# martius-lab/iCEM

Measured on AMD Instinct MI355X. Metric: traj-steps/sec (N x h), iCEM inner planning loop, higher is better.
Workload: dtype f32 storage; model step 2xfp16 planes (3 products), f32 accumulate

## Files before the change

### icem_amd/csrc/fused_dev.h

```cpp
#pragma once
#include "icem_fused.h"

#include <climits>
#include <cmath>
#include <cstdlib>
#include <algorithm>
#include <type_traits>
#include <utility>

#include "exchange_dev.h"
#include "philox.h"
#include "refit.h"

#ifndef ICEM_FAST_SHAPES
#define ICEM_FAST_SHAPES(X) X(30, 6, 17) X(30, 6, 18) X(12, 6, 17) X(13, 4, 17) X(30, 17, 24)
#endif
#define ICEM_FAST_HORIZONS(X) X(30) X(12) X(13) X(10)

namespace icem {

namespace {

constexpr int HMAX = 32;
constexpr int SWG = 256;
// ... 1459 lines not shown
        n_cand += (unsigned)__popcll(m);
    }
    __builtin_amdgcn_fence(__ATOMIC_SEQ_CST, "workgroup");
    if (n_cand <= 64) {
        unsigned long long key = lane < (int)n_cand ? lds_reread_u64(&cand[lane]) : KEY_SENTINEL;
        key = wave_sort_n(key, lane, n_cand);
        if (lane < a.K) sel[lane] = key;
    } else {
        for (int r = 0; r < a.K; ++r) {
            unsigned long long head = k[0];
#pragma unroll
            for (int j = 1; j < 5; ++j) head = k[j] < head ? k[j] : head;
            const unsigned long long best = wave_min_u64(head);
            if (best != KEY_SENTINEL) {
#pragma unroll
                for (int j = 0; j < 5; ++j)
                    if (k[j] == best) k[j] = KEY_SENTINEL;
            }
            if (lane == 0) sel[r] = best;
        }
    }
}

template <int NW>
__device__ __forceinline__ bool merge_select_split_by_rank(const MergeSingleArgs& a) { return a.n_keep <= (16 - a.K) * NW; }
template <int NW>
__device__ __forceinline__ float merge_keep_cost_split(const MergeSingleArgs& a, int lane, int w) {
    const int j = w + NW * (lane - a.K);
    return a.elites_cost_cur ? a.elites_cost_cur[(lane >= a.K && lane < 16 && j < a.n_keep) ? j : 0] : 0.f;
}
template <int NW>
__device__ __forceinline__ void merge_select_split_keep(const MergeSingleArgs& a, int lane, int w, unsigned long long* wsel,
                                                        unsigned long long* sel, float keep_cost) {
    if (lane >= a.K && lane < 16) {
        const int j = w + NW * (lane - a.K);
        wsel[w * 16 + lane] = (j < a.n_keep && a.elites_cost_cur) ? make_key(keep_cost, keep_index0(a) + j) : KEY_SENTINEL;
    }
    if (w == 0 && lane < 16) sel[lane] = KEY_SENTINEL;
}
template <int NW>
__device__ __forceinline__ void merge_select_split_rank(const MergeSingleArgs& a, int lane, int w, const unsigned long long* wsel,
                                                        unsigned long long* sel) {
    typedef unsigned long long u64x2 __attribute__((ext_vector_type(2)));
    const int i = lane & 15, q = lane >> 4;
    const unsigned long long mine = wsel[w * 16 + i];
    const u64x2* pairs = reinterpret_cast<const u64x2*>(wsel) + q;
    unsigned place = 0;
#pragma unroll
    for (int c = 0; c < 2 * NW; ++c) {
        const u64x2 b = pairs[4 * c];
        place += (b[0] < mine ? 1u : 0u) + (b[1] < mine ? 1u : 0u);
    }
    place += (unsigned)__shfl_xor((int)place, 16, 64);
    place += (unsigned)__shfl_xor((int)place, 32, 64);
    if (q == 0 && mine != KEY_SENTINEL && place < (unsigned)a.K) sel[place] = mine;
}

template <int KREG, bool REC>
__device__ __forceinline__ void merge_rows(const MergeSingleArgs& a, const unsigned long long* sel, const int* slot,
                                           const float* (&rows)[KREG]) {
    const int hd = a.h * a.d;
    const int lane = (int)(threadIdx.x & 63);
    const int v = REC ? slot[lane < a.K ? lane : 0] : key_idx(sel[lane < a.K ? lane : 0]);
    const float* mine;
    if (REC) mine = v < a.n_rec ? a.records + (size_t)v * (hd + 2) + 2 : a.elites_cur + (size_t)(v - a.n_rec) * hd;
    else mine = v < a.n_pool ? a.actions + (size_t)v * hd : a.elites_cur + (size_t)(v - a.n_global) * hd;
    typedef const float __attribute__((address_space(1))) * GRow;
    const unsigned long long bits = (unsigned long long)(size_t)mine;
#pragma unroll
    for (int r = 0; r < KREG; ++r) {
        const int rr = r < a.K ? r : 0;
        const unsigned lo = (unsigned)__builtin_amdgcn_readlane((int)(unsigned)bits, rr);
        const unsigned hi = (unsigned)__builtin_amdgcn_readlane((int)(unsigned)(bits >> 32), rr);
        rows[r] = (const float*)reinterpret_cast<GRow>((size_t)(((unsigned long long)hi << 32) | lo));
    }
}

template <int H, int D, int ROUNDS, bool RAW>
__device__ __forceinline__ void sample_into_tile(const FastSampleArgs& sa, int n_rows, int r_mine, int jd, float* trow,
                                                 const float* mrow) {
    constexpr int HD = H * D;
    if (r_mine < sa.n) {
        if (RAW) {
            sample_row<H, ROUNDS>(sa.W, (unsigned)(sa.first_index + r_mine), (unsigned)jd, sa.off_lo, sa.off_hi,
                                  sa.seed_lo, sa.seed_hi, [&](int t, float y) { trow[t * D] = y; }, sa.white != 0);
        } else {
            const float lo = sa.low[jd], hi = sa.high[jd];
            sample_row<H, ROUNDS>(sa.W, (unsigned)(sa.first_index + r_mine), (unsigned)jd, sa.off_lo, sa.off_hi,
                                  sa.seed_lo, sa.seed_hi, [&](int t, float y) {
                                      const float v = __builtin_fmaf(y, mrow[HD + t * D], mrow[t * D]);
                                      trow[t * D] = __builtin_amdgcn_fmed3f(v, lo, hi);
                                  }, sa.white != 0);
        }
    } else if (r_mine < n_rows && !RAW) {
        const int e = r_mine - sa.n;
        const float lo = sa.low[jd], hi = sa.high[jd];
        float last = 0.f;
        sample_row<H, ROUNDS>(sa.W, (unsigned)e, (unsigned)jd, sa.off2_lo, sa.off2_hi, sa.seed_lo, sa.seed_hi,
                              [&](int t, float y) {
                                  if (t == H - 1) {
                                      const float v = __builtin_fmaf(y, mrow[HD + t * D], mrow[t * D]);
                                      last = __builtin_amdgcn_fmed3f(v, lo, hi);
                                  }
                              }, sa.white != 0);
        const float* src = sa.elites_src + (size_t)e * HD + jd;
        for (int t = 0; t < H - 1; ++t) trow[t * D] = src[(t + 1) * D];
        trow[(H - 1) * D] = last;
    } else {
        for (int t = 0; t < H; ++t) trow[t * D] = 0.f;
    }
}

template <int H, int D, int ROUNDS, bool RAW, typename Publish>
__device__ __forceinline__ void sample_into_tile_quad(const FastSampleArgs& sa, bool live, int n_rows, int r_mine, int jd, int q,
                                                      float* trow, const float* mrow, const float* Wl, Publish&& publish) {
    constexpr int HD = H * D;
    float g[HMAX];
    const int kind = !live ? 3 : (r_mine < sa.n ? 0 : ((r_mine < n_rows && !RAW) ? 1 : 2));
    if (kind == 0)
        row_normals_quad<H, ROUNDS>((unsigned)(sa.first_index + r_mine), (unsigned)jd, sa.off_lo, sa.off_hi, sa.seed_lo, sa.seed_hi, q, g);
    else if (kind == 1)
        row_normals_quad<H, ROUNDS>((unsigned)(r_mine - sa.n), (unsigned)jd, sa.off2_lo, sa.off2_hi, sa.seed_lo, sa.seed_hi, q, g);
    publish();
    if (kind == 0) {
        if (RAW) {
            row_synth_quad<H>(Wl, g, q, [&](int t, float y) { trow[t * D] = y; }, sa.white != 0);
        } else {
            const float lo = sa.low[jd], hi = sa.high[jd];
            row_synth_quad<H>(Wl, g, q, [&](int t, float y) {
                const float v = __builtin_fmaf(y, mrow[HD + t * D], mrow[t * D]);
                trow[t * D] = __builtin_amdgcn_fmed3f(v, lo, hi);
            }, sa.white != 0);
        }
    } else if (kind == 1) {
        const int e = r_mine - sa.n;
        const float lo = sa.low[jd], hi = sa.high[jd];
        row_synth_quad<H>(Wl, g, q, [&](int t, float y) {
            if (t == H - 1) {
                const float v = __builtin_fmaf(y, mrow[HD + t * D], mrow[t * D]);
                trow[(H - 1) * D] = __builtin_amdgcn_fmed3f(v, lo, hi);
            }
        }, sa.white != 0);
        const float* src = sa.elites_src + (size_t)e * HD + jd;
        for (int t = q; t < H - 1; t += 4) trow[t * D] = src[(t + 1) * D];
    } else if (kind == 2) {
        for (int t = q; t < H; t += 4) trow[t * D] = 0.f;
    }
}

__device__ __forceinline__ void note_nonfinite(const FastRolloutArgs& a, float cost, bool stored) {
    if (stored && cost != cost) atomicAdd(a.nonfinite, 1u);
}

template <typename Tile, int H, int D, bool PLANES_FIRST = false>
__device__ __forceinline__ unsigned long long rollout_slab(Tile& tile, const FastRolloutArgs& ra, const float* rd0, int row,
                                                           int n_rows, unsigned long long run_key, bool first, int lane) {
    const bool live = row < n_rows;
    typename Tile::State st;
    tile.init(st);
    if constexpr (PLANES_FIRST && Tile::LONE_STEP) {
        float raw[2] = {rd0[tile.xoff[0]], rd0[tile.xoff[1]]};
#pragma unroll
        for (int t = 0; t < H; ++t) tile.step_lone(st, raw, rd0 + (t + 1 < H ? t + 1 : t) * D);
    } else {
#pragma unroll
        for (int t = 0; t < H; ++t) tile.template step<PLANES_FIRST>(st, rd0 + t * D);
    }
    const float cost = tile.cost(st);
    if (live && lane < 16) ra.costs[row] = cost;
    note_nonfinite(ra, cost, live && lane < 16);
    if (ra.K > 0) {
        const unsigned long long key = (lane < 16 && live && row < ra.n_cand) ? make_key(cost, row) : KEY_SENTINEL;
        run_key = topk_push16(run_key, key, first, ra.K, lane);
    }
    return run_key;
}

template <typename TileT, int H, int D>
struct StreamT {
    using Tile = TileT;
    static constexpr int HD = H * D;
    static constexpr int VW = HD % 4 == 0 ? 4 : 2;
    static_assert(HD % 2 == 0, "8-byte aligned action rows");
    using Vec = typename VecOf<VW>::type;
    static constexpr int TC = r16_chunk_steps(H, D, VW);
    static_assert(TC > 0, "no aligned action chunk for this (H, D)");
    static constexpr int CB = TC * D;
    static constexpr int C4 = CB / VW;
    static constexpr int CBP = (C4 % 2) ? CB : CB + VW;
    static constexpr int NCH = H / TC;
    static constexpr int F4 = 16 * C4;
    static constexpr int NLD = (F4 + 63) / 64;
    static constexpr int STG = Tile::SLACK + 16 * CBP + Tile::TAIL;

    int ld_row[NLD], ld_c4[NLD];
    bool ld_on[NLD];
    const float* rd0;
    float* stage;

    __device__ __forceinline__ void init(const Tile& tile, float* stage_buf, int lane) {
        stage = stage_buf;
        rd0 = tile.read_ptr(stage_buf, lane, CBP);
#pragma unroll
        for (int m = 0; m < NLD; ++m) {
            const int f = m * 64 + lane;
            ld_on[m] = f < F4;
            ld_row[m] = ld_on[m] ? f / C4 : 0;
            ld_c4[m] = ld_on[m] ? f % C4 : 0;
        }
    }

    __device__ __forceinline__ unsigned long long run(const Tile& tile, const FastRolloutArgs& a, int tile_id, int lane,
                                                      unsigned long long run_key, bool first, Vec (&pre)[NLD]) const {
        const int row = tile_id * 16 + (lane & 15);
        const bool live = row < a.n_rows;
        const Vec* src[NLD];
#pragma unroll
        for (int m = 0; m < NLD; ++m) {
            const int r = tile_id * 16 + ld_row[m];
            src[m] = reinterpret_cast<const Vec*>(a.actions + (size_t)(r < a.n_rows ? r : 0) * HD) + ld_c4[m];
        }
        typename Tile::State st;
        tile.init(st);
#pragma unroll
        for (int t = 0; t < H; ++t) {
            if (t % TC == 0) {
#pragma unroll
                for (int m = 0; m < NLD; ++m)
                    if (ld_on[m]) *reinterpret_cast<Vec*>(&stage[Tile::SLACK + ld_row[m] * CBP + VW * ld_c4[m]]) = pre[m];
                if (t / TC + 1 < NCH) {
#pragma unroll
                    for (int m = 0; m < NLD; ++m) pre[m] = src[m][(t / TC + 1) * C4];
                }
            }
            tile.step(st, rd0 + (t % TC) * D);
        }
        const float cost = tile.cost(st);
        if (live && lane < 16) a.costs[row] = cost;
        note_nonfinite(a, cost, live && lane < 16);
        if (a.K > 0) {
            const unsigned long long key = (lane < 16 && live && row < a.n_cand) ? make_key(cost, row) : KEY_SENTINEL;
            run_key = topk_push16(run_key, key, first, a.K, lane);
        }
        return run_key;
    }

    __device__ __forceinline__ void first_loads(const float* pool, int n_rows, int tile_id, Vec (&pre)[NLD]) const {
#pragma unroll
        for (int m = 0; m < NLD; ++m) {
            const int r = tile_id * 16 + ld_row[m];
            pre[m] = (reinterpret_cast<const Vec*>(pool + (size_t)(r < n_rows ? r : 0) * HD) + ld_c4[m])[0];
        }
    }
    __device__ __forceinline__ unsigned long long run_xf(const Tile& tile, const FastRolloutArgs& a, float* pool, int n_xf,
                                                         bool row0_mean, bool store_back, const float* dist, float lo, float hi, int tile_id,
                                                         int lane, unsigned long long run_key, bool first, Vec (&pre)[NLD]) const {
        const int row = tile_id * 16 + (lane & 15);
        const bool live = row < a.n_rows;
        unsigned voff[NLD];
        bool xf_on[NLD], is0[NLD], st_on[NLD];
#pragma unroll
        for (int m = 0; m < NLD; ++m) {
            const int r = tile_id * 16 + ld_row[m];
            voff[m] = (unsigned)(r < a.n_rows ? r : 0) * (unsigned)HD + (unsigned)(VW * ld_c4[m]);
            xf_on[m] = ld_on[m] && r < a.n_rows && r < n_xf;
            is0[m] = xf_on[m] && row0_mean && r == 0;
            st_on[m] = xf_on[m] && store_back;
        }
        typename Tile::State st;
        tile.init(st);
        float xraw[2] = {0.f, 0.f};
#pragma unroll
        for (int t = 0; t < H; ++t) {
            if (t % TC == 0) {
                const int ch = t / TC;
#pragma unroll
                for (int m = 0; m < NLD; ++m) {
                    asm volatile("" ::: "memory");
                    const int eo = ch * CB + VW * ld_c4[m];
                    const Vec mu = *reinterpret_cast<const Vec*>(dist + eo);
                    const Vec sg = *reinterpret_cast<const Vec*>(dist + HD + eo);
                    float y[VW], vm[VW], vs[VW];
                    __builtin_memcpy(y, &pre[m], sizeof(Vec));
                    __builtin_memcpy(vm, &mu, sizeof(Vec));
                    __builtin_memcpy(vs, &sg, sizeof(Vec));
#pragma unroll
                    for (int k = 0; k < VW; ++k) {
                        const float v = __builtin_amdgcn_fmed3f(__builtin_fmaf(y[k], vs[k], vm[k]), lo, hi);
                        y[k] = xf_on[m] ? (is0[m] ? vm[k] : v) : y[k];
                    }
                    Vec out;
                    __builtin_memcpy(&out, y, sizeof(Vec));
                    if (ld_on[m]) *reinterpret_cast<Vec*>(&stage[Tile::SLACK + ld_row[m] * CBP + VW * ld_c4[m]]) = out;
                    if (ch + 1 < NCH) pre[m] = *reinterpret_cast<const Vec*>(pool + voff[m] + (ch + 1) * CB);
                    if (st_on[m]) *reinterpret_cast<Vec*>(pool + voff[m] + ch * CB) = out;
                }
                asm volatile("" ::: "memory");
                if constexpr (Tile::LONE_STEP) { xraw[0] = rd0[tile.xoff[0]]; xraw[1] = rd0[tile.xoff[1]]; }
            }
            if constexpr (Tile::LONE_STEP) tile.step_lone(st, xraw, rd0 + ((t + 1) % TC ? (t + 1) % TC : t % TC) * D);
            else tile.step(st, rd0 + (t % TC) * D);
        }
        const float cost = tile.cost(st);
        if (live && lane < 16) a.costs[row] = cost;
        note_nonfinite(a, cost, live && lane < 16);
        if (a.K > 0) {
            const unsigned long long key = (lane < 16 && live && row < a.n_cand) ? make_key(cost, row) : KEY_SENTINEL;
            run_key = topk_push16(run_key, key, first, a.K, lane);
        }
        return run_key;
    }
};
template <int H, int D, int O, int KIND, int ARITH = 0>
using Stream16 = StreamT<typename TileSel<H, D, O, KIND, ARITH>::type, H, D>;

template <int KREG>
// ... 99 lines not shown
```

### icem_amd/csrc/icem_fused.h

```cpp
#pragma once
#include <hip/hip_runtime.h>
#include <stdint.h>
#include <cstddef>
#include <cstring>
#include <vector>
#include "cost_args.h"
#include "options.h"

namespace icem {

constexpr int FAST_MAX_LISTS = 256;
struct BatchHint;
struct LaunchCtx;

constexpr int XCHG_MAX_WORLD = 16;
struct XchgWait {
    const unsigned* flags = nullptr;
    unsigned* status = nullptr;
    unsigned seq = 0;
    int world = 0;
    unsigned max_polls = 0;
    const void* records = nullptr;
};
struct XchgPush {
    unsigned char* const* peers = nullptr;
    size_t rec_byte_off = 0;
    int world = 0;
    int flag_idx = 0;
    unsigned seq = 0;
};

struct FastSampleArgs {
    int n, h, d;
    long long first_index;
    const float* W;
    const float* mean;
    const float* std;
    const float* low;
    const float* high;
    uint32_t seed_lo, seed_hi, off_lo, off_hi;
    int row0_mean;
    float* out;
    int n_shift;
    const float* elites_src;
    uint32_t off2_lo, off2_hi;
    int white;
    const float* raw_src = nullptr;
};
bool fast_sample_supported(int h, int d);
void launch_sample_folded(const LaunchCtx& cx, const FastSampleArgs& a, int rounds);

struct FastRolloutArgs {
    int n_rows;
    int n_cand;
    int K;
    int o;
    int cost_mode;
    const float* Mp;
    const int* perm;
    const float* obs0;
    float ctrl_w, lin_w, flip_pen, flip_th;
    int flip_col;
    const float* actions;
    float* costs;
    float* part_c;
    int* part_i;
    unsigned long long* part_k;
    int list_wgs = 0;
    long long* dbg;
    int arith = 0;
    float act_mag = 1.f;
    float m_scale = 1.f, b_scale = 1.f;
    unsigned* nonfinite = nullptr;
};
bool fast_rollout_supported(int h, int d, int O, int K);
void launch_rollout16(const FastRolloutArgs& a, int h, int d, int O, int kind, hipStream_t st);
int rollout_lists(int h, int d, int O, int n_rows);

template <typename T> struct CostArgs;
bool hn_rollout_supported(int h, int d, int o, int K);
int hn_rollout_lists(const BatchHint& bh, int n_rows);
int hn_tail_rows(const BatchHint& bh, int n_rows, int n_tail);
struct WideCost {
    int lin_idx, flip_idx;
    float ctrl_w, lin_w, flip_pen, flip_th;
};
struct HnArgs {
    FastRolloutArgs r;
    const float* A;
    const float* B;
    int lda, ldb;
    WideCost wc;
    const CostArgs<float>* cs;
};
bool hn_cost_program(int n32, int n4, int np, int* prog);
void launch_rollout_hn(const LaunchCtx& cx, const FastRolloutArgs& r, int h, int d, int o, int kind, const float* A, int lda, const float* B, int ldb,
                       int lin_idx, int flip_idx, const CostArgs<float>* cs, const int* prog);

struct WideRolloutArgs {
    int n_rows, n_cand, K;
    int o, d, h;
    int kb, xs;
    int planes;
    float minv;
    const float* ksc;
    const float* csc;
    float sbound;
    int cost_mode;
    int lin_idx, flip_idx;
    float ctrl_w, lin_w, flip_pen, flip_th;
    const CostArgs<float>* cs;
    long long* dbg;
    const float* Mp;
    const float* obs0;
    const float* actions;
    float* costs;
    float* part_c;
    int* part_i;
    unsigned long long* part_k;
};
bool wide_rollout_supported(int o, int d, int K);
bool gemm_rollout_supported(int o, int d, int K);
int wide_rollout_lists(int n_rows);
int wide_kb(int o, int d);
int wide_xs(int o, int d);
void pack_wide_model(int o, int d, const double* A, const double* B, std::vector<float>& Mp);
void launch_rollout_wide(const WideRolloutArgs& a, int kind, hipStream_t st);
int wide_split_kb(int o, int d);
int wide_split_xs(int o, int d);
int wide_split_lists(int n_rows);
bool wide_split_fits(int o, int d);
int wide_model_imbalance_log2(int o, int d, const double* A, const double* B);
void pack_wide_model_split(int o, int d, const double* A, const double* B, int planes, std::vector<unsigned short>& Mb, float* minv,
                           std::vector<float>* ksc, std::vector<float>* csc, float* sbound);
void launch_rollout_wide_split(const WideRolloutArgs& a, int kind, hipStream_t st);
void launch_rollout_rows_wide(const WideRolloutArgs& a, int row0, int n_tail, const float* A, const float* B, int kind,
                              hipStream_t st);

struct MergeSingleArgs {
    int n_lists;
    int n_keep;
    int keep_base = -1;
    int n_pool;
    int n_global;
    int K, h, d, last;
    float alpha, init_std;
    const unsigned long long* part_k;
    const float* records;
    int n_rec;
    XchgWait xw;
    const float* actions;
    const float* elites_cur;
    const float* elites_cost_cur;
    float* elites_next;
    float* elites_cost_next;
    const float* mean;
    const float* std;
    float* mean_out;
    float* std_out;
    const float* low;
    const float* high;
    float* executed;
    float* best_cost;
    long long* dbg;
    int n_raw = 0;
    float xf_lo = 0.f, xf_hi = 0.f;
};
void launch_merge_single(const LaunchCtx& cx, const MergeSingleArgs& a);
bool merge_noise_ok(const MergeSingleArgs& a, int rounds);
void launch_merge_noise(const LaunchCtx& cx, const MergeSingleArgs& a, const FastSampleArgs& z, const FastSampleArgs& z2);
struct UpdateSmallArgs {
    const float* costs;
    const float* pool;
    const float* keep_costs;
    const float* keep_actions;
    int n, n_keep, K, hd;
    float alpha;
    float* mean;
    float* std;
    float* elites_out;
    float* elite_costs_out;
    int* idx_out;
};
void launch_update_small(const UpdateSmallArgs& a, hipStream_t st);
constexpr int UPDATE_FINISH_MAX_HD = 256;
struct UpdateFinishArgs {
    UpdateSmallArgs u;
    int d;
    float init_std;
    const float* low;
    const float* high;
    float* executed;
    float* best_cost;
    float* result;
};
void launch_update_small_batch(const UpdateFinishArgs* args_dev, int n, bool finish, hipStream_t st);
bool topk_small_ok(int n, int K);
void launch_topk_small(const float* costs, int n, int K, float* out_c, int* out_i, hipStream_t st);
bool pack_can_push(int K, int h, int d);
void launch_pack_records(const MergeSingleArgs& a, int n_loc, int shard_lo, float* records, hipStream_t st,
                         const XchgPush& px = XchgPush());
void launch_pack_merge(const MergeSingleArgs& pk, int n_loc, int shard_lo, float* records, const XchgPush& px, const MergeSingleArgs& m,
                       hipStream_t st);

struct PackPrev {
    const unsigned long long* part_k = nullptr;
    const float* actions = nullptr;
    int n_lists = 0, n_pool = 0, n_global = 0, K = 0;
    int n_loc = 0, shard_lo = 0;
    int n_keep = 0;
    const float* keep_costs = nullptr;
    float* records = nullptr;
    XchgPush px;
    float* pub = nullptr;
    unsigned* pub_flag = nullptr;
    unsigned pub_seq = 0;
};
bool sample_rollout_pack_ok(const BatchHint& bh, int h, int d, int O, int rounds, int n_rows, int K);
bool sample_folded_pack_ok(int h, int d, int rounds, int K);

void launch_noise_rows(const FastSampleArgs& a, int rounds, hipStream_t st);
struct IterAheadArgs {
    FastRolloutArgs r;
    MergeSingleArgs m;
    int has_merge;
    int n_xf;
// ... 167 lines not shown
```

### icem_amd/csrc/k_iter_small.hip

```cpp
#include "fused_dev.h"

namespace icem {

namespace {

constexpr bool sr_quad(int d, int rw) { return rw <= 2 && ((4 * 16 * rw * d + 63) / 64) * 64 + 64 <= 1024; }
constexpr int sr_threads(int d, int rw) { return (((sr_quad(d, rw) ? 4 : 1) * 16 * rw * d + 63) / 64) * 64; }

template <int H, int D, int O, int KIND, int ROUNDS, int RW, int KREG, bool REC, int ARITH>
__device__ __forceinline__ void sample_rollout_body(const FastSampleArgs& sa, const FastRolloutArgs& ra, const MergeSingleArgs& am,
                                                    const PackPrev& ap) {
    constexpr bool PM = KREG > 0;
    constexpr bool QS = sr_quad(D, RW);
    constexpr bool T4 = QS && O <= 20 && sr_threads(D, RW) >= 256 * RW && ARITH == 0;
    using T16 = typename TileSel<H, D, O, KIND, ARITH>::type;
    using Tile = typename std::conditional<T4, Tile4<H, D, (O <= 20 ? O : 17), KIND>, T16>::type;
    constexpr int RWV = T4 ? 4 * RW : RW;
    constexpr int HD = H * D;
    constexpr int TPB = 16 * RW;
    constexpr int ROWS = TPB * D;
    constexpr int NT = sr_threads(D, RW);
    constexpr int NTT = NT + (PM ? 64 : 0);
    static_assert(NTT <= 1024 && HD % 2 == 0, "workgroup shape");
    constexpr int VW = HD % 4 == 0 ? 4 : 2;
    using Vec = typename VecOf<VW>::type;
    __shared__ __attribute__((aligned(16))) float ms[2 * HD];
    __shared__ __attribute__((aligned(16))) float tilebuf[T16::SLACK + TPB * HD + T16::TAIL];
    __shared__ unsigned long long wg_keys[2][RW][32];
    __shared__ float obs_stage[32];
    constexpr int WROWS = H / 2 + 1;
    __shared__ __attribute__((aligned(16))) float Wl[QS ? NT / 64 : 1][QS ? WROWS * WQ_STRIDE : 4];
    __shared__ unsigned long long sel[PM ? 64 : 1];
    __shared__ unsigned long long cand[PM ? 64 : 1];
    __shared__ int slot[PM ? 64 : 1];
    float* tile_rows = tilebuf + T16::SLACK;
    const int tid = threadIdx.x;
    const int lane = tid & 63;
    const int wave = tid >> 6;
    const int n_rows = ra.n_rows;
    const bool has_pack = PM && REC && ap.part_k != nullptr;
    if constexpr (PM && REC) {
        if (has_pack && blockIdx.x == 0) {
            MergeSingleArgs pk{};
            pk.n_lists = ap.n_lists;
            pk.n_pool = ap.n_pool;
            pk.n_global = ap.n_global;
            pk.K = ap.K;
            pk.h = H;
            pk.d = D;
            pk.part_k = ap.part_k;
            pk.actions = ap.actions;
            pk.n_keep = ap.n_keep;
            pk.elites_cost_cur = ap.keep_costs;
            pk.keep_base = ap.n_loc;
            __builtin_amdgcn_s_setprio(3);
            if (ra.dbg && tid == 0) ra.dbg[0] = wall_clock64();
            if (tid < 64) {
                if constexpr (NTT <= 512)
                    merge_select<12>(pk, lane, cand, sel);
                else
                    merge_select_stream(pk, lane, cand, sel);
            }
            __syncthreads();
            if (ra.dbg && tid == 0) ra.dbg[1] = wall_clock64();
            pack_records_body<12>(pk, ap.n_loc, ap.shard_lo, ap.records, ap.px, tilebuf, sel, tid, NTT);
            if (ra.dbg && tid == 0) ra.dbg[2] = wall_clock64();
            return;
        }
    }
    const int wg = blockIdx.x - (has_pack ? 1 : 0);
    const int n_wg = ra.list_wgs > 0 ? ra.list_wgs : (int)gridDim.x - (has_pack ? 1 : 0);
    const int base = wg * TPB;
    if (base >= n_rows) return;
    if (ra.dbg && tid == 0 && wg == 0) ra.dbg[8] = wall_clock64();
    const int rowi = QS ? tid >> 2 : tid, q = tid & 3;
    const int nl = rowi / D, jd = rowi - nl * D;
    const bool has_row = rowi < ROWS;
    float* trow = tile_rows + nl * HD + jd;
    const float* mrow = ms + jd;
    Tile tile;
    float obs_reg = 0.f;
    constexpr int WPL = (WROWS * HMAX + 63) / 64;
    float wreg[QS ? WPL : 1];
    const bool pre_drawn = !PM && sa.raw_src != nullptr;
    if constexpr (QS) {
        if (tid < NT && !pre_drawn) {
#pragma unroll
            for (int i = 0; i < WPL; ++i) wreg[i] = sa.W[(i * 64 + lane) < WROWS * HMAX ? i * 64 + lane : 0];
        }
    }
    const int r_mine = base + nl;
    float lo_reg = 0.f, hi_reg = 0.f;
    if ((PM || pre_drawn) && tid < NT) {
        lo_reg = sa.low[jd];
        hi_reg = sa.high[jd];
    }
    constexpr int NVR = !PM ? (TPB * (HD / VW) + NTT - 1) / NTT : 1;
    constexpr int NVB = NVR < 4 ? NVR : 4;
    constexpr int NEL = !PM && QS ? (H - 1 + 3) / 4 : 1;
    typedef float RawV __attribute__((ext_vector_type(VW)));
    RawV rawv[NVB];
    float elv[NEL];
    if (!PM) {
        const int total4 = (n_rows - base < TPB ? n_rows - base : TPB) * (HD / VW);
        RawV* t4 = reinterpret_cast<RawV*>(tile_rows);
        float mreg[(HD + NTT - 1) / NTT], sreg[(HD + NTT - 1) / NTT];
#pragma unroll
        for (int i = 0; i < (HD + NTT - 1) / NTT; ++i) {
            const int e = tid + i * NTT;
            mreg[i] = sa.mean[e < HD ? e : 0];
            sreg[i] = sa.std[e < HD ? e : 0];
        }
        if (pre_drawn) {
            const RawV* g4 = reinterpret_cast<const RawV*>(sa.raw_src + (size_t)base * HD);
#pragma unroll
            for (int i = 0; i < NVB; ++i) {
                const int e = tid + i * NTT;
                rawv[i] = g4[e < total4 ? e : 0];
            }
            if constexpr (QS) {
                if (has_row && tid < NT && r_mine >= sa.n && r_mine < n_rows) {
                    const float* src = sa.elites_src + (size_t)(r_mine - sa.n) * HD + jd;
#pragma unroll
                    for (int i = 0; i < NEL; ++i) elv[i] = src[(q + 4 * i < H - 1 ? q + 4 * i + 1 : 1) * D];
                }
            }
        }
        obs_reg = ra.obs0[(tid < 32 && tid < ra.o) ? tid : 0];
        if (wave < RWV) tile.load(ra, lane);
#pragma unroll
        for (int i = 0; i < (HD + NTT - 1) / NTT; ++i) {
            const int e = tid + i * NTT;
            if (e < HD) {
                ms[e] = mreg[i];
                ms[HD + e] = sreg[i];
            }
        }
        if (pre_drawn) {
#pragma unroll
            for (int i = 0; i < NVB; ++i) {
                const int e = tid + i * NTT;
                if (e < total4) t4[e] = rawv[i];
            }
            if constexpr (NVR > NVB) {
                const RawV* g4 = reinterpret_cast<const RawV*>(sa.raw_src + (size_t)base * HD);
                for (int e0 = tid + NVB * NTT; e0 < total4; e0 += NVB * NTT) {
#pragma unroll
                    for (int i = 0; i < NVB; ++i) rawv[i] = g4[e0 + i * NTT < total4 ? e0 + i * NTT : 0];
#pragma unroll
                    for (int i = 0; i < NVB; ++i)
                        if (e0 + i * NTT < total4) t4[e0 + i * NTT] = rawv[i];
                }
            }
        }
        __syncthreads();
    }
    if (ra.dbg && tid == 0 && wg == 0) ra.dbg[9] = wall_clock64();
    if (pre_drawn) {
        if (has_row && tid < NT) {
            const float lo = lo_reg, hi = hi_reg;
            constexpr int QN = QS ? 4 : 1;
            const int q0 = QS ? q : 0;
            if (r_mine < sa.n) {
                for (int t = q0; t < H; t += QN) {
                    const float v = __builtin_fmaf(trow[t * D], mrow[HD + t * D], mrow[t * D]);
                    trow[t * D] = __builtin_amdgcn_fmed3f(v, lo, hi);
                }
            } else if (r_mine < n_rows) {
                const float* src = sa.elites_src + (size_t)(r_mine - sa.n) * HD + jd;
                if ((H - 1) % QN == q0) {
                    const float v = __builtin_fmaf(trow[(H - 1) * D], mrow[HD + (H - 1) * D], mrow[(H - 1) * D]);
                    trow[(H - 1) * D] = __builtin_amdgcn_fmed3f(v, lo, hi);
                }
                if constexpr (QS) {
#pragma unroll
                    for (int i = 0; i < NEL; ++i)
                        if (q + 4 * i < H - 1) trow[(q + 4 * i) * D] = elv[i];
                } else {
                    for (int t = q0; t < H - 1; t += QN) trow[t * D] = src[(t + 1) * D];
                }
            } else {
                for (int t = q0; t < H; t += QN) trow[t * D] = 0.f;
            }
        }
    } else
    if constexpr (QS) {
        if (tid < NT) {
            float* wl = Wl[wave];
            sample_into_tile_quad<H, D, ROUNDS, PM>(sa, has_row, n_rows, r_mine, jd, q, trow, mrow, wl, [&]() {
#pragma unroll
                for (int i = 0; i < WPL; ++i) {
                    const int e = i * 64 + lane;
                    if (e < WROWS * HMAX) wl[(e / HMAX) * WQ_STRIDE + (e % HMAX)] = wreg[i];
                }
                __builtin_amdgcn_fence(__ATOMIC_RELEASE, "wavefront");
                __builtin_amdgcn_wave_barrier();
                __builtin_amdgcn_fence(__ATOMIC_ACQUIRE, "wavefront");
            });
        }
    } else if (has_row) {
        sample_into_tile<H, D, ROUNDS, PM>(sa, n_rows, r_mine, jd, trow, mrow);
    }
    if constexpr (PM) {
        if (tid >= NT) {
            if constexpr (RW <= 4) __builtin_amdgcn_s_setprio(3);
            if constexpr (REC) {
                if (ra.dbg && lane == 0 && wg == 0) ra.dbg[3] = wall_clock64();
            }
            else if constexpr (RW >= 8)
                merge_select_stream(am, lane, cand, sel);
            else
                merge_select_shallow<3>(am, lane, cand, sel);
        }
    }
    if (PM) {
        obs_reg = ra.obs0[(tid < 32 && tid < ra.o) ? tid : 0];
        if (wave < RWV) tile.load(ra, lane);
    }
    const float* rd0 = nullptr;
    if constexpr (!T4) rd0 = tile.read_ptr(tilebuf + (wave < RW ? wave : 0) * 16 * HD, lane, HD);
    if constexpr (PM) {
        const MergeSingleArgs& m = am;
        if constexpr (REC) {
            merge_select_records_wg(am, tid >= NT, lane, tid, NTT, sel, slot, (ra.dbg && wg == 0) ? ra.dbg + 7 : nullptr);
            if (ra.dbg && tid == 0 && wg == 0) ra.dbg[4] = wall_clock64();
        } else {
            __syncthreads();
        }
        if (ra.dbg && tid == 0 && wg == 0) ra.dbg[5] = wall_clock64();
        if (!REC && ra.dbg && tid == 0 && wg == 0) ra.dbg[15] = wall_clock64();
        const float* rows[KREG > 0 ? KREG : 1];
        merge_rows<KREG, REC>(m, sel, slot, rows);
        for (int e = tid; e < HD; e += NTT) {
            float xs[KREG > 0 ? KREG : 1];
#pragma unroll
            for (int r = 0; r < KREG; ++r) xs[r] = rows[r][e];
            float nm, ns;
            refit_element_regs<float, KREG>(m.K, m.alpha, m.mean[e], m.std[e], xs, nm, ns);
            ms[e] = nm;
            ms[HD + e] = ns;
            if (wg == 0) {
                m.mean_out[e] = nm;
                m.std_out[e] = ns;
#pragma unroll
                for (int r = 0; r < KREG; ++r)
                    if (r < m.K) m.elites_next[(size_t)r * HD + e] = xs[r];
            }
        }
        if (wg == 0 && tid < m.K) m.elites_cost_next[tid] = key_cost(sel[tid]);
        __syncthreads();
        if (ra.dbg && tid == 0 && wg == 0) ra.dbg[6] = wall_clock64();
        if (!REC && ra.dbg && tid == 0 && wg == 0) ra.dbg[7] = wall_clock64();
        if (has_row && r_mine < sa.n) {
            const float lo = lo_reg, hi = hi_reg;
            for (int t = QS ? q : 0; t < H; t += QS ? 4 : 1) {
                const float v = __builtin_fmaf(trow[t * D], mrow[HD + t * D], mrow[t * D]);
                trow[t * D] = __builtin_amdgcn_fmed3f(v, lo, hi);
            }
        }
    }
    if (tid < 32) {
        float ov = obs_reg;
        asm volatile("" : "+v"(ov));
        obs_stage[tid] = tid < ra.o ? ov : 0.f;
    }
    if (ra.dbg && tid == 0 && wg == 0) ra.dbg[10] = wall_clock64();
    __syncthreads();
    if (sa.row0_mean && sa.first_index + base == 0) {
        for (int e = tid; e < HD; e += NTT) tile_rows[e] = ms[e];
        __syncthreads();
    }
    {
        const int total4 = (n_rows - base < TPB ? n_rows - base : TPB) * (HD / VW);
        const Vec* t4 = reinterpret_cast<const Vec*>(tile_rows);
        Vec* g4 = reinterpret_cast<Vec*>(sa.out + (size_t)base * HD);
        constexpr int CP0 = (NTT - 64 * RWV >= 128) ? 64 * RWV : 0;
        if (tid >= CP0)
            for (int e = tid - CP0; e < total4; e += NTT - CP0) g4[e] = t4[e];
    }
    if (ra.dbg && tid == 0 && wg == 0) ra.dbg[11] = wall_clock64();
    unsigned long long run_key = KEY_SENTINEL;
    if constexpr (T4) {
        if (wave < RWV) {
            tile.load_obs(obs_stage);
            const int rs = wave * 4 + (lane >> 4);
            const int row = base + rs;
            const float* rd = tile.read_ptr(tilebuf, rs, HD);
            const float* ar = tile.row_ptr(tilebuf, rs, HD);
            typename Tile::State st;
            tile.init(st);
#pragma unroll
            for (int t = 0; t < H; ++t) tile.step(st, rd + t * D, ar + t * D);
            const float cost = tile.cost(st);
            const bool live = row < n_rows;
            if ((lane & 15) == 0) {
                if (live) ra.costs[row] = cost;
                note_nonfinite(ra, cost, live);
                wg_keys[0][0][rs] = (live && row < ra.n_cand) ? make_key(cost, row)
                                    : TPB <= 16 ? KEY_SENTINEL : ((KEY_SENTINEL & 0xFFFFFFFF00000000ull) | (KEY_FILL_LO + (unsigned)rs));
            }
        }
        if (ra.dbg && tid == 0 && wg == 0) ra.dbg[13] = wall_clock64();
        if (ra.K > 0 && wg < n_wg) {
            __syncthreads();
            if (wave == 0 && TPB <= 16) {
                const unsigned long long key = wave_sort_first<16>(lane < TPB ? wg_keys[0][0][lane] : KEY_SENTINEL, lane);
                if (lane < ra.K) {
                    if (ra.part_k) {
                        ra.part_k[(size_t)lane * n_wg + wg] = key;
                    } else {
                        ra.part_c[(size_t)wg * ra.K + lane] = key_cost(key);
                        ra.part_i[(size_t)wg * ra.K + lane] = key_idx(key);
                    }
                }
            } else if (wave == 0) {
                constexpr int NK = TPB <= 16 ? 16 : 32, PARTS = 64 / NK, PER = NK / PARTS;
                static_assert(TPB <= 32 && PER % 2 == 0, "one wave counts for the slab");
                const unsigned long long* keys = &wg_keys[0][0][0];
                const int i = lane & (NK - 1), part = lane / NK;
                const unsigned long long mine = i < TPB ? keys[i] : KEY_SENTINEL;
                unsigned place = 0;
#pragma unroll
                for (int c = 0; c < PER; ++c) {
                    const int e = part * PER + c;
                    place += (e < TPB && keys[e < TPB ? e : 0] < mine) ? 1u : 0u;
                }
                if (NK == 16) place += (unsigned)__shfl_xor((int)place, 16, 64);
                place += (unsigned)__shfl_xor((int)place, 32, 64);
                if (part == 0 && i < TPB && place < (unsigned)ra.K) {
                    const bool filler = (mine >> 32) == (KEY_SENTINEL >> 32) && (unsigned)mine >= KEY_FILL_LO;
                    const unsigned long long key = filler ? KEY_SENTINEL : mine;
                    if (ra.part_k) {
                        ra.part_k[(size_t)place * n_wg + wg] = key;
                    } else {
                        ra.part_c[(size_t)wg * ra.K + place] = key_cost(key);
                        ra.part_i[(size_t)wg * ra.K + place] = key_idx(key);
                    }
                }
            }
        }
    } else {
        if (wave < RW) {
            tile.load_obs(obs_stage);
            run_key = rollout_slab<Tile, H, D, true>(tile, ra, rd0, base + wave * 16 + (lane & 15), n_rows, run_key, true, lane);
            if (ra.dbg && tid == 0 && wg == 0) ra.dbg[12] = wall_clock64();
        }
        if (ra.dbg && tid == 0 && wg == 0) ra.dbg[13] = wall_clock64();
        if (ra.K > 0 && wg < n_wg) wg_merge_emit<RW>(wg_keys, run_key, ra.K, lane, wave, ra, wg, n_wg);
    }
    if (ra.dbg && tid == 0 && wg == 0) ra.dbg[14] = wall_clock64();
}


template <int H, int D, int O, int KIND, int ROUNDS, int RW, int KREG, bool REC, int ARITH>
__global__ __launch_bounds__(sr_threads(D, RW) + (KREG > 0 ? 64 : 0)) void sample_rollout_kernel(FastIterArgs a) {
    sample_rollout_body<H, D, O, KIND, ROUNDS, RW, KREG, REC, ARITH>(a.s, a.r, a.m, a.p);
}

template <int H, int D, int O, int KIND, int ROUNDS, int RW, int KREG, int ARITH>
__global__ __launch_bounds__(sr_threads(D, RW) + (KREG > 0 ? 64 : 0)) void sample_rollout_batch_kernel(const FastIterArgs* __restrict__ args,
                                                                                                      BatchBases bases) {
    const FastIterArgs& a = args[blockIdx.y];
    FastSampleArgs s = from_device(a.s);
    const unsigned long long base = bases.v[blockIdx.y];
    add_base64(s.off_lo, s.off_hi, base);
    add_base64(s.off2_lo, s.off2_hi, base);
    const FastRolloutArgs r = from_device(a.r);
    const MergeSingleArgs m = from_device(a.m);
    sample_rollout_body<H, D, O, KIND, ROUNDS, RW, KREG, false, ARITH>(s, r, m, a.p);
}

}

constexpr int single_launch_max_rw(int h, int d) {
    int best = 0;
    for (int rw = 1; rw <= 8; rw *= 2)
        if (sr_threads(d, rw) + 64 <= 1024 && 16 * rw * h * d * 4 <= 120 * 1024) best = rw;
    return best;
}

static bool sample_rollout_shape(const BatchHint& bh, int h, int d, int O, int rounds, int n_rows, int n_tail, int* grid_out, int* rw_out,
                                 int* tail_out = nullptr) {
    const int max_rw = opt_i(OPT_FUSE_MAX_RW);
    int grid, rw, tail = 0;
    r16_shape(n_rows, &grid, &rw);
    const int mult = bh.mult;
    if (mult > 1) {
        int g_all, rw_all;
        r16_shape(n_rows * mult, &g_all, &rw_all);
        const int cap = opt_i(OPT_BATCH_MAX_RW);
        rw = std::min(std::max(rw, rw_all), std::min(cap > 0 ? cap : 8, single_launch_max_rw(h, d)));
        while (rw > 1 && rw > single_launch_max_rw(h, d)) rw /= 2;
        grid = (std::max(1, (n_rows + 15) / 16) + rw - 1) / rw;
        if (grid > FAST_MAX_LISTS) return false;
    } else
    if (n_tail > 0 && n_tail <= 64) {
        int g2, w2;
        r16_shape(n_rows - n_tail, &g2, &w2);
        if (w2 < rw && sr_threads(d, w2) + 64 <= 512 && g2 == FAST_MAX_LISTS && n_rows - n_tail == FAST_MAX_LISTS * 16 * w2) {
            rw = w2;
            tail = n_tail;
        }
    }
    if (rounds != 10 || rw > max_rw || n_rows <= 0 || !fast_rollout_supported(h, d, O, 1) || !fast_sample_supported(h, d))
        return false;
    if (rw > single_launch_max_rw(h, d)) return false;
    *grid_out = tail ? (n_rows + 16 * rw - 1) / (16 * rw) : std::min(grid, (n_rows + 16 * rw - 1) / (16 * rw));
    *rw_out = rw;
    if (tail_out) *tail_out = tail;
    return true;
}

int sample_rollout_lists(const BatchHint& bh, int h, int d, int O, int rounds, int n_rows, int n_tail, int* tail_out) {
    int grid, rw, tail = 0;
    if (!sample_rollout_shape(bh, h, d, O, rounds, n_rows, n_tail, &grid, &rw, &tail)) return 0;
    if (tail_out) *tail_out = tail;
    return tail ? FAST_MAX_LISTS : grid;
}

bool sample_rollout_merge_ok(const BatchHint& bh, int h, int d, int O, int rounds, int n_rows, int K) {
    const int on = opt_i(OPT_MERGE_PROLOGUE);
    int grid, rw;
    return on && K + 1 <= 12 && sample_rollout_shape(bh, h, d, O, rounds, n_rows, 0, &grid, &rw);
}

bool sample_rollout_pack_ok(const BatchHint& bh, int h, int d, int O, int rounds, int n_rows, int K) {
    const int on = opt_i(OPT_RIDING_PACK);
    int grid, rw;
    return on && sample_rollout_merge_ok(bh, h, d, O, rounds, n_rows, K) && sample_rollout_shape(bh, h, d, O, rounds, n_rows, 0, &grid, &rw) &&
           K * (h * d + 2) <= 16 * rw * h * d;
}

namespace {
template <int H, int D, int O, int KIND, int RW, int KREG, bool REC, int ARITH>
struct SrInst {
    static constexpr int THREADS = sr_threads(D, RW) + (KREG > 0 ? 64 : 0);
    static constexpr bool BATCHED = !REC;
    static void solo(int grid, hipStream_t st, const FastIterArgs& a) {
        hipLaunchKernelGGL((sample_rollout_kernel<H, D, O, KIND, 10, RW, KREG, REC, ARITH>), dim3(grid), dim3(THREADS), 0, st, a);
    }
    static void batch(int grid, int n, hipStream_t st, const FastIterArgs* args_dev, const BatchBases& bases) {
        hipLaunchKernelGGL((sample_rollout_batch_kernel<H, D, O, KIND, 10, RW, KREG, ARITH>), dim3(grid, n), dim3(THREADS), 0, st, args_dev, bases);
    }
};
template <int H, int D, int O, int RW, class F>
bool sample_rollout_pick(const LaunchKey& k, F& f) {
    if constexpr (RW > single_launch_max_rw(H, D)) {
        return false;
    } else {
        if (k.waves != RW) return false;
        auto with = [&](auto kind, auto arith) {
            constexpr int KK = decltype(kind)::value, AA = decltype(arith)::value;
            if (k.form == 2) f(SrInst<H, D, O, KK, RW, 12, true, AA>{});
            else if (k.form == 1) f(SrInst<H, D, O, KK, RW, 12, false, AA>{});
            else f(SrInst<H, D, O, KK, RW, 0, false, AA>{});
            return true;
        };
        using I0 = std::integral_constant<int, 0>;
        using I1 = std::integral_constant<int, 1>;
        if constexpr (O <= 20) {
            if (k.arith == 1) return k.kind == 1 ? with(I1{}, I1{}) : with(I0{}, I1{});
        }
        return k.kind == 1 ? with(I1{}, I0{}) : with(I0{}, I0{});
    }
}
template <class F>
bool sample_rollout_dispatch(const LaunchKey& k, F&& f) {
#define XR(HH, DD, OO)                                                                                      \
    if (k.h == HH && k.d == DD && k.O == OO)                                                                \
        return sample_rollout_pick<HH, DD, OO, 1>(k, f) || sample_rollout_pick<HH, DD, OO, 2>(k, f) ||      \
               sample_rollout_pick<HH, DD, OO, 4>(k, f) || sample_rollout_pick<HH, DD, OO, 8>(k, f);
    ICEM_FAST_SHAPES(XR)
#undef XR
    return false;
}
}

void launch_sample_rollout(const LaunchCtx& cx, const FastIterArgs& a, int h, int d, int O, int kind, bool merge_prologue) {
    LaunchKey k;
    if (!sample_rollout_shape(cx.hint, h, d, O, 10, a.r.n_rows, a.r.list_wgs > 0 ? a.s.n_shift : 0, &k.wgs[0], &k.waves)) return;
    k.family = LAUNCH_SAMPLE_ROLLOUT;
    k.h = h, k.d = d, k.O = O, k.kind = kind, k.arith = a.r.arith;
    k.form = !merge_prologue ? 0 : a.m.records ? 2 : 1;
    k.wgs[1] = (k.form == 2 && a.p.part_k) ? 1 : 0;
    submit(cx, k, k.form != 2, [&](void* dst, unsigned long long base) { batch_form(a, base, dst); },
           [&] { sample_rollout_dispatch(k, [&](auto inst) { inst.solo(k.wgs[0] + k.wgs[1], cx.st, a); }); });
}

void launch_sample_rollout_batch(const LaunchKey& k, const FastIterArgs* args_dev, const BatchBases& bases, int n, hipStream_t st) {
    sample_rollout_dispatch(k, [&](auto inst) {
        if constexpr (decltype(inst)::BATCHED) inst.batch(k.wgs[0], n, st, args_dev, bases);
    });
}

}
```

### icem_amd/csrc/options.h

```cpp
#pragma once

namespace icem {

#define ICEM_OPTIONS(X)                                                                                                   \
    X(DISABLE_FAST, "disable_fast", 0.0)              \
    X(FUSE_MAX_RW, "fuse_max_rw", 8.0)                \
    X(MERGE_PROLOGUE, "merge_prologue", 1.0)                                      \
    X(RIDING_PACK, "riding_pack", 1.0)                             \
    X(PUBLISHED_MERGE, "published_merge", 1.0)             \
    X(PACK_MERGE, "pack_merge", 1.0)                  \
    X(NOISE_AHEAD, "noise_ahead", 1.0)                             \
    X(NOISE_AHEAD_MIN_ROWS, "noise_ahead_min_rows", 0.0)                                                                \
    X(NOISE_AHEAD_SHARDED, "noise_ahead_sharded", 1.0)                                                                     \
    X(AHEAD_STAMPS, "ahead_stamps", 0.0)                                                                                   \
    X(AHEAD_TAIL_FRAC, "ahead_tail_frac", 0.4)                                                                             \
    X(AHEAD_NEXT1_FRAC, "ahead_next1_frac", 0.3)                                                                           \
    X(AHEAD_NOISE_LDS_KB, "ahead_noise_lds_kb", -1.0)                                                                      \
    X(PREDRAW, "predraw", 1.0)                              \
    X(GK_SAMPLE, "gk_sample", 1.0)                          \
    X(GK_ROLLOUT_THREAD, "gk_rollout_thread", 0.0)                   \
    X(GK_SELECT, "gk_select", 1.0)                                    \
    X(HN_PAIR, "hn_pair", 1.0)                                                               \
    X(HN_SPLIT, "hn_split", 1.0)                                                                                           \
    X(RSSM_SPLIT, "rssm_split", 1.0)                                                                                       \
    X(RSSM_SPLIT_MAX_N, "rssm_split_max_n", 65536.0)                                                                       \
    X(RSSM_SPLIT_TT, "rssm_split_tt", 0.0)                                                                                 \
    X(BATCH_AHEAD, "batch_ahead", 1.0)                \
    X(BATCH_AHEAD_MIN_ROWS, "batch_ahead_min_rows", 49152.0)    \
    X(BATCH_MAX_RW, "batch_max_rw", 0.0)              \
    X(LEARNED_STEP, "learned_step", 1.0)              \
    X(XCHG_LOOPBACK, "xchg_loopback", 0.0)            \
    X(XCHG_MAX_POLLS, "xchg_max_polls", 0.0)
enum Opt {
#define X(id, name, def) OPT_##id,
    ICEM_OPTIONS(X)
#undef X
    OPT_COUNT
};
double opt(Opt k);
inline int opt_i(Opt k) { return (int)opt(k); }

}
```

Baseline: 7.645 billion.

## Pipeline merge-prologue refit with rollout via helper waves and staged barriers

For the H=30, D=6, O=17 fp16-plane shape, the fused sample-rollout kernel now splits the merge/refit prologue across helper waves. Each helper wave handles whole timesteps, and helpers are grouped into blocks that release their columns to the rollout wave through staggered __syncthreads placed inside the rollout step loop. The rollout wave can then begin stepping early timesteps while later timesteps are still being refit and sampled, instead of waiting for the whole prologue. This adds barrier coordination, option knobs for block count, stagger and priority, and a tight shape-specific code path with matching barrier counts that must stay consistent.

```diff
diff --git a/icem_amd/csrc/fused_dev.h b/icem_amd/csrc/fused_dev.h
--- a/icem_amd/csrc/fused_dev.h
+++ b/icem_amd/csrc/fused_dev.h
@@ -1635,16 +1635,24 @@
     if (stored && cost != cost) atomicAdd(a.nonfinite, 1u);
 }
 
-template <typename Tile, int H, int D, bool PLANES_FIRST = false>
+struct NoStepHook {
+    __device__ __forceinline__ void operator()(int) const {}
+};
+template <typename Tile, int H, int D, bool PLANES_FIRST = false, typename Before = NoStepHook>
 __device__ __forceinline__ unsigned long long rollout_slab(Tile& tile, const FastRolloutArgs& ra, const float* rd0, int row,
-                                                           int n_rows, unsigned long long run_key, bool first, int lane) {
+                                                           int n_rows, unsigned long long run_key, bool first, int lane,
+                                                           Before&& before = Before{}) {
     const bool live = row < n_rows;
     typename Tile::State st;
     tile.init(st);
     if constexpr (PLANES_FIRST && Tile::LONE_STEP) {
+        before(-1);
         float raw[2] = {rd0[tile.xoff[0]], rd0[tile.xoff[1]]};
 #pragma unroll
-        for (int t = 0; t < H; ++t) tile.step_lone(st, raw, rd0 + (t + 1 < H ? t + 1 : t) * D);
+        for (int t = 0; t < H; ++t) {
+            before(t);
+            tile.step_lone(st, raw, rd0 + (t + 1 < H ? t + 1 : t) * D);
+        }
     } else {
 #pragma unroll
         for (int t = 0; t < H; ++t) tile.template step<PLANES_FIRST>(st, rd0 + t * D);
diff --git a/icem_amd/csrc/icem_fused.h b/icem_amd/csrc/icem_fused.h
--- a/icem_amd/csrc/icem_fused.h
+++ b/icem_amd/csrc/icem_fused.h
@@ -72,6 +72,7 @@
     float act_mag = 1.f;
     float m_scale = 1.f, b_scale = 1.f;
     unsigned* nonfinite = nullptr;
+    int pipe_wpb = 0;
 };
 bool fast_rollout_supported(int h, int d, int O, int K);
 void launch_rollout16(const FastRolloutArgs& a, int h, int d, int O, int kind, hipStream_t st);
diff --git a/icem_amd/csrc/k_iter_small.hip b/icem_amd/csrc/k_iter_small.hip
--- a/icem_amd/csrc/k_iter_small.hip
+++ b/icem_amd/csrc/k_iter_small.hip
@@ -6,6 +6,7 @@
 
 constexpr bool sr_quad(int d, int rw) { return rw <= 2 && ((4 * 16 * rw * d + 63) / 64) * 64 + 64 <= 1024; }
 constexpr int sr_threads(int d, int rw) { return (((sr_quad(d, rw) ? 4 : 1) * 16 * rw * d + 63) / 64) * 64; }
+constexpr int sr_helper_waves(int d, int rw) { return sr_threads(d, rw) / 64; }
 
 template <int H, int D, int O, int KIND, int ROUNDS, int RW, int KREG, bool REC, int ARITH>
 __device__ __forceinline__ void sample_rollout_body(const FastSampleArgs& sa, const FastRolloutArgs& ra, const MergeSingleArgs& am,
@@ -38,6 +39,14 @@
     const int lane = tid & 63;
     const int wave = tid >> 6;
     const int n_rows = ra.n_rows;
+    constexpr int NHW = sr_helper_waves(D, RW);
+    constexpr bool PIPE_OK = PM && !REC && RW == 1 && !T4 && QS && ARITH == 1 && H == 30 && D == 6 && O == 17;
+    constexpr int EPW = PIPE_OK ? HD / NHW : 1, TPW = PIPE_OK ? EPW / D : 1;
+    static_assert(!PIPE_OK || (EPW * NHW == HD && TPW * D == EPW && 2 * EPW <= 64), "whole timesteps per helper wave, two rows per pass");
+    const int pipe_wpb = PIPE_OK ? (ra.pipe_wpb & 0xFF) : 0;
+    const int pipe_stagger = PIPE_OK ? ((ra.pipe_wpb >> 8) & 0xFF) : 0;
+    const bool pipe_prio = PIPE_OK && ((ra.pipe_wpb >> 16) & 1);
+    const int uwave = __builtin_amdgcn_readfirstlane((int)(threadIdx.x >> 6));
     const bool has_pack = PM && REC && ap.part_k != nullptr;
     if constexpr (PM && REC) {
         if (has_pack && blockIdx.x == 0) {
@@ -95,6 +104,14 @@
         lo_reg = sa.low[jd];
         hi_reg = sa.high[jd];
     }
+    const int pe_l = PIPE_OK ? (lane < 2 * EPW ? lane % EPW : 0) : 0;
+    float plo = 0.f, phi = 0.f;
+    if constexpr (PIPE_OK) {
+        if (pipe_wpb > 0 && uwave > 0) {
+            plo = sa.low[pe_l % D];
+            phi = sa.high[pe_l % D];
+        }
+    }
     constexpr int NVR = !PM ? (TPB * (HD / VW) + NTT - 1) / NTT : 1;
     constexpr int NVB = NVR < 4 ? NVR : 4;
     constexpr int NEL = !PM && QS ? (H - 1 + 3) / 4 : 1;
@@ -230,6 +247,69 @@
         if (ra.dbg && tid == 0 && wg == 0) ra.dbg[5] = wall_clock64();
         if (!REC && ra.dbg && tid == 0 && wg == 0) ra.dbg[15] = wall_clock64();
         const float* rows[KREG > 0 ? KREG : 1];
+        if (pipe_wpb > 0) {
+          if constexpr (PIPE_OK) {
+            if (uwave == 0) {
+                if (lane < 32) {
+                    float ov = obs_reg;
+                    asm volatile("" : "+v"(ov));
+                    obs_stage[lane] = lane < ra.o ? ov : 0.f;
+                }
+                __builtin_amdgcn_fence(__ATOMIC_RELEASE, "wavefront");
+                __builtin_amdgcn_wave_barrier();
+                __builtin_amdgcn_fence(__ATOMIC_ACQUIRE, "wavefront");
+            } else {
+                const int hw = uwave - 1, blk = hw / pipe_wpb, n_blk = NHW / pipe_wpb;
+                const bool act = lane < 2 * EPW;
+                const int par = lane >= EPW ? 1 : 0;
+                const int e = hw * EPW + pe_l;
+                if (pipe_prio) __builtin_amdgcn_s_setprio(0);
+                for (int i = 0; i < blk * pipe_stagger; ++i) __builtin_amdgcn_s_sleep(1);
+                merge_rows<KREG, REC>(m, sel, slot, rows);
+                float xs[KREG > 0 ? KREG : 1];
+#pragma unroll
+                for (int r = 0; r < KREG; ++r) xs[r] = rows[r][e];
+                const float om = m.mean[e], os = m.std[e];
+                for (int i = 0; i < blk; ++i) __syncthreads();
+                float* col = tile_rows + e;
+                float y[TPB / 2];
+#pragma unroll
+                for (int i = 0; i < TPB / 2; ++i) y[i] = col[(2 * i + par) * HD];
+                float nm, ns;
+                refit_element_regs<float, KREG>(m.K, m.alpha, om, os, xs, nm, ns);
+                if (act && par == 0) {
+                    ms[e] = nm;
+                    ms[HD + e] = ns;
+                }
+                if (act) {
+                    const bool row0 = sa.row0_mean && sa.first_index + base == 0;
+#pragma unroll
+                    for (int i = 0; i < TPB / 2; ++i) {
+                        const int rl = 2 * i + par;
+                        const float v = __builtin_amdgcn_fmed3f(__builtin_fmaf(y[i], ns, nm), plo, phi);
+                        col[rl * HD] = (row0 && rl == 0) ? nm : (base + rl < sa.n ? v : y[i]);
+                    }
+                }
+                if (ra.dbg && wg == 0 && tid == NTT - 64) ra.dbg[7] = wall_clock64();
+                for (int i = blk; i < n_blk; ++i) {
+                    __syncthreads();
+                    if (i == blk && wg == 0 && act && par == 0) {
+                        m.mean_out[e] = nm;
+                        m.std_out[e] = ns;
+#pragma unroll
+                        for (int r = 0; r < KREG; ++r)
+                            if (r < m.K) m.elites_next[(size_t)r * HD + e] = xs[r];
+                    }
+                }
+                if (wg == 0 && hw == 0 && lane < m.K) m.elites_cost_next[lane] = key_cost(sel[lane]);
+                const int total4 = (n_rows - base < TPB ? n_rows - base : TPB) * (HD / VW);
+                const Vec* t4 = reinterpret_cast<const Vec*>(tile_rows);
+                Vec* g4 = reinterpret_cast<Vec*>(sa.out + (size_t)base * HD);
+                for (int i = tid - 64; i < total4; i += NTT - 64) g4[i] = t4[i];
+                if (ra.dbg && wg == 0 && tid == NTT - 64) ra.dbg[11] = wall_clock64();
+            }
+          }
+        } else {
         merge_rows<KREG, REC>(m, sel, slot, rows);
         for (int e = tid; e < HD; e += NTT) {
             float xs[KREG > 0 ? KREG : 1];
@@ -258,7 +338,9 @@
                 trow[t * D] = __builtin_amdgcn_fmed3f(v, lo, hi);
             }
         }
-    }
+        }
+    }
+    if (pipe_wpb == 0) {
     if (tid < 32) {
         float ov = obs_reg;
         asm volatile("" : "+v"(ov));
@@ -279,6 +361,7 @@
             for (int e = tid - CP0; e < total4; e += NTT - CP0) g4[e] = t4[e];
     }
     if (ra.dbg && tid == 0 && wg == 0) ra.dbg[11] = wall_clock64();
+    }
     unsigned long long run_key = KEY_SENTINEL;
     if constexpr (T4) {
         if (wave < RWV) {
@@ -342,7 +425,19 @@
     } else {
         if (wave < RW) {
             tile.load_obs(obs_stage);
-            run_key = rollout_slab<Tile, H, D, true>(tile, ra, rd0, base + wave * 16 + (lane & 15), n_rows, run_key, true, lane);
+            run_key = rollout_slab<Tile, H, D, true>(tile, ra, rd0, base + wave * 16 + (lane & 15), n_rows, run_key, true, lane, [&](int t) {
+                if constexpr (PIPE_OK) {
+                    if (t < 0) {
+                        if (pipe_wpb > 0) {
+                            if (pipe_prio) __builtin_amdgcn_s_setprio(3);
+                            __syncthreads();
+                            if (ra.dbg && tid == 0 && wg == 0) ra.dbg[10] = wall_clock64();
+                        }
+                    } else if ((t + 1) % TPW == 0 && t + 1 < H) {
+                        if (pipe_wpb > 0 && ((t + 1) / TPW) % pipe_wpb == 0) __syncthreads();
+                    }
+                }
+            });
             if (ra.dbg && tid == 0 && wg == 0) ra.dbg[12] = wall_clock64();
         }
         if (ra.dbg && tid == 0 && wg == 0) ra.dbg[13] = wall_clock64();
@@ -483,8 +578,12 @@
     k.h = h, k.d = d, k.O = O, k.kind = kind, k.arith = a.r.arith;
     k.form = !merge_prologue ? 0 : a.m.records ? 2 : 1;
     k.wgs[1] = (k.form == 2 && a.p.part_k) ? 1 : 0;
-    submit(cx, k, k.form != 2, [&](void* dst, unsigned long long base) { batch_form(a, base, dst); },
-           [&] { sample_rollout_dispatch(k, [&](auto inst) { inst.solo(k.wgs[0] + k.wgs[1], cx.st, a); }); });
+    const int nb = opt_i(OPT_PROLOGUE_PIPELINE);
+    const bool piped = k.form == 1 && k.waves == 1 && k.arith == 1 && h == 30 && d == 6 && O == 17 && nb > 0 && sr_helper_waves(6, 1) % nb == 0;
+    FastIterArgs b = a;
+    b.r.pipe_wpb = piped ? (sr_helper_waves(6, 1) / nb) | ((opt_i(OPT_PROLOGUE_STAGGER) & 0xFF) << 8) | (opt_i(OPT_PROLOGUE_PRIO) ? 1 << 16 : 0) : 0;
+    submit(cx, k, k.form != 2, [&](void* dst, unsigned long long base) { batch_form(b, base, dst); },
+           [&] { sample_rollout_dispatch(k, [&](auto inst) { inst.solo(k.wgs[0] + k.wgs[1], cx.st, b); }); });
 }
 
 void launch_sample_rollout_batch(const LaunchKey& k, const FastIterArgs* args_dev, const BatchBases& bases, int n, hipStream_t st) {
diff --git a/icem_amd/csrc/options.h b/icem_amd/csrc/options.h
--- a/icem_amd/csrc/options.h
+++ b/icem_amd/csrc/options.h
@@ -16,6 +16,9 @@
     X(AHEAD_TAIL_FRAC, "ahead_tail_frac", 0.4)                                                                             \
     X(AHEAD_NEXT1_FRAC, "ahead_next1_frac", 0.3)                                                                           \
     X(AHEAD_NOISE_LDS_KB, "ahead_noise_lds_kb", -1.0)                                                                      \
+    X(PROLOGUE_PIPELINE, "prologue_pipeline", 3.0)    \
+    X(PROLOGUE_STAGGER, "prologue_stagger", 0.0)      \
+    X(PROLOGUE_PRIO, "prologue_prio", 0.0)            \
     X(PREDRAW, "predraw", 1.0)                              \
     X(GK_SAMPLE, "gk_sample", 1.0)                          \
     X(GK_ROLLOUT_THREAD, "gk_rollout_thread", 0.0)                   \
```

After: 7.509 billion. 1.8% lower.
